# NVIDIA-NeMo/NeMo

Measured on AMD Instinct MI355X. Metric: audio-sec/s training throughput, Conformer-CTC-Large @ 1/2/4/8 MI355X, higher is better.
Workload: dtype bf16; 1 GPU; Conformer-CTC-Large bf16, batch=32x20s synthetic 16 kHz clips per GPU, 1xMI355X (BASELINE.json configs[1]); global_batch=32, parallelism=dp1

## Files before the change

nemo_amd/csrc/attention.hip:

```cpp
#include <stdlib.h>
#include "common.h"
#include "mi355x_asr.h"

typedef __attribute__((address_space(3))) void lds_void_t;
typedef const __attribute__((address_space(1))) void glb_void_t;
typedef __attribute__((ext_vector_type(4))) short s16x4;
typedef __attribute__((address_space(3))) s16x4 lds_s16x4_t;

typedef __attribute__((address_space(3))) const char lds_cchar_t;
__device__ __forceinline__ uint32_t lds_addr(const void* p) { return (uint32_t)(uintptr_t)(lds_cchar_t*)p; }

__device__ __forceinline__ void dma16(const void* src, const void* lds_base) {
  asm volatile("s_mov_b32 m0, %1\n\ts_nop 0\n\tglobal_load_lds_dwordx4 %0, off"
               :
               : "v"(src), "s"(__builtin_amdgcn_readfirstlane(lds_addr(lds_base)))
               : "memory");
}

__device__ __forceinline__ void dma4(const void* src, const void* lds_base) {
  asm volatile("s_mov_b32 m0, %1\n\ts_nop 0\n\tglobal_load_lds_dword %0, off"
               :
               : "v"(src), "s"(__builtin_amdgcn_readfirstlane(lds_addr(lds_base)))
               : "memory");
}

#define ABQ 128
#define ABK 32
#define ABAND (ABQ + ABK)
#define SG_LD 66
#define APRING 6

__device__ __forceinline__ uint32_t attn_key(const DropCfg& d, int b, int h) {
  return mix32(mix32(d.key ^ (uint32_t)(b * 0x632BE5AB)) + (uint32_t)h * 0x9E3779B9u);
}
#define ADROP_G 0x9E3779B9u
#define ADROP_KA 0x2C1B3Du
#define ADROP_KB 0x5A2D39u
__device__ __forceinline__ uint32_t adrop_rcode(uint32_t akey, uint32_t bi) { return mix32(akey + bi * 0x9E3779B9u); }
__device__ __forceinline__ uint32_t adrop_ccode(uint32_t bj) { return mix32(bj * 0x85EBCA6Bu + 0x165667B1u); }
__device__ __forceinline__ uint32_t adrop_seed(uint32_t x) { return __umul24(x, 0x846CA7u) + (x >> 13); }
__device__ __forceinline__ uint32_t adrop_y(uint32_t t) { return t ^ (t >> 15); }
__device__ __forceinline__ bool attn_keep(const DropCfg& d, uint32_t akey, int i, int j) {
  if (d.threshold == 0u) return true;
  const uint32_t seed = adrop_seed(adrop_rcode(akey, (uint32_t)i >> 2) ^ adrop_ccode((uint32_t)j >> 2));
  const uint32_t y = adrop_y(seed + (uint32_t)((i & 3) * 2 + ((j & 3) >> 1)) * ADROP_G);
  return __umul24(y, (j & 1) ? ADROP_KB : ADROP_KA) >= d.threshold;
}
__device__ __forceinline__ float attn_drop(const DropCfg& d, uint32_t akey, int i, int j) {
  return attn_keep(d, akey, i, j) ? d.scale : 0.f;
}

template <int ADK>
__device__ __forceinline__ int a_off(int r, int chunk) { return r * ADK + ((chunk ^ ((r >> 1) & 7)) << 3); }

template <int ADK>
__device__ __forceinline__ void stage_rows(const bf16_t* base, long long ld, int row0, int rmax, bf16_t* lds, int nchunks) {
  constexpr int NCH = ADK / 8;
  const int wave = threadIdx.x >> 6;
  for (int q0 = 0; q0 < nchunks; q0 += 256) {
    const int q = q0 + threadIdx.x;
    if (q0 + wave * 64 < nchunks) {
      const int r = q / NCH, ck = q % NCH;
      const int gck = ck ^ ((r >> 1) & 7);
      int gr = row0 + r;
      gr = gr < 0 ? 0 : (gr > rmax ? rmax : gr);
      const bf16_t* src = base + __mul24(gr, (int)ld) + gck * 8;
      bf16_t* dst = lds + (q0 + wave * 64) * 8;
      dma16(src, dst);
    }
  }
}
template <int ADK>
__device__ __forceinline__ void stage_v(const bf16_t* base, long long ld, int row0, int rmax, bf16_t* lds) {
  constexpr int NCH = ADK / 8;
  const int wave = threadIdx.x >> 6;
#pragma unroll
  for (int q0 = 0; q0 < 32 * NCH; q0 += 256) {
    const int q = q0 + threadIdx.x;
    const int k = q / NCH, cp = q % NCH;
    const int c = cp ^ ((k & 3) << 1);
    int gr = row0 + k;
    gr = gr > rmax ? rmax : gr;
    const bf16_t* src = base + __mul24(gr, (int)ld) + c * 8;
    bf16_t* dst = lds + (q0 + wave * 64) * 8;
    dma16(src, dst);
  }
}
template <int ADK>
__device__ __forceinline__ bf16x8 vt_frag(const bf16_t* vt, int dv0, int s, int lane) {
  const int t = lane & 15, g4 = (lane >> 4) & 1, lh = lane >> 5;
  const int col = dv0 + g4 * 16 + (t & 3) * 4;
  union { bf16x8 v; s16x4 h[2]; } u;
#pragma unroll
  for (int r = 0; r < 2; ++r) {
    const int krow = 16 * s + 8 * r + 4 * lh + (t >> 2);
    const int off = krow * ADK + (((col >> 3) ^ ((krow & 3) << 1)) << 3) + (col & 7);
    u.h[r] = __builtin_amdgcn_ds_read_tr16_b64_v4i16((lds_s16x4_t*)(vt + off));
  }
  return u.v;
}

__device__ __forceinline__ bf16x8 pack8(const float* v) {
  union { bf16x8 v; uint32_t w[4]; } u;
#pragma unroll
  for (int j = 0; j < 4; ++j) u.w[j] = pack_bf2(v[2 * j], v[2 * j + 1]);
  return u.v;
}

template <int NKK>
__device__ __forceinline__ void load_q(const bf16_t* qrow, const float* bias, bf16x8 (&out)[NKK], bool valid, int lh) {
#pragma unroll
  for (int kk = 0; kk < NKK; ++kk) {
    float v[8];
    const int k0 = kk * 16 + lh * 8;
    if (valid) {
      const u32x4 t = *reinterpret_cast<const u32x4*>(qrow + k0);
#pragma unroll
      for (int j = 0; j < 4; ++j) { v[2 * j] = __uint_as_float(t[j] << 16); v[2 * j + 1] = __uint_as_float(t[j] & 0xffff0000u); }
#pragma unroll
      for (int j = 0; j < 8; ++j) v[j] += bias[k0 + j];
    } else {
#pragma unroll
      for (int j = 0; j < 8; ++j) v[j] = 0.f;
    }
    out[kk] = pack8(v);
  }
}

template <int ADK>
__global__ __launch_bounds__(256, ADK == 64 ? 2 : 1) void relpos_flash_fwd_kernel(const bf16_t* __restrict__ qkv, long long ldq,
                                                                  const bf16_t* __restrict__ pos, long long ldp,
                                                                  const float* __restrict__ bias_u, const float* __restrict__ bias_v,
                                                                  const long long* __restrict__ len, bf16_t* __restrict__ ctx,
                                                                  bf16_t* __restrict__ ctx_lo, long long ldo,
                                                                  float* __restrict__ lse, int B, int H, int T,
                                                                  int Tp, float scale, DropCfg drop,
                                                                  const long long* __restrict__ cu) {
  drop_resolve(drop);
  constexpr int NKK = ADK / 16, NDT = ADK / 32, NCH = ADK / 8;
  __shared__ __attribute__((aligned(16))) bf16_t s_k2[2][ABK * ADK];
  __shared__ __attribute__((aligned(16))) bf16_t s_v2[2][ABK * ADK];
  __shared__ __attribute__((aligned(16))) bf16_t s_p[APRING * 32 * ADK];
  __shared__ __attribute__((aligned(16))) float s_g[4][32 * SG_LD];

  const int b = blockIdx.z, h = blockIdx.y;
  const int i0_blk = blockIdx.x * ABQ;
  const int lane = threadIdx.x & 63, wave = __builtin_amdgcn_readfirstlane(threadIdx.x >> 6);
  const int q = lane & 31, lh = lane >> 5;
  const int i = i0_blk + wave * 32 + q;
  const int L = (int)min((long long)T, len[b]);
  const bool qvalid = i < L;
  const int P = 2 * T - 1;
  const long long row0 = cu ? cu[b] : (long long)b * T;
  const int Tr = cu ? L : T;
  const int Trc = Tr > 0 ? Tr - 1 : 0;

  if (cu && i0_blk >= L) {
    if (lse && lh == 0 && i < T) lse[((long long)b * H + h) * T + i] = 0.f;
    return;
  }
  const bf16_t* qbase = qkv + row0 * ldq + h * ADK;
  const bf16_t* kbase = qbase + (ldq / 3);
  const bf16_t* vbase = qbase + 2 * (ldq / 3);
  const bf16_t* pbase = pos + h * ADK;

  bf16x8 qu[NKK], qv[NKK];
  load_q<NKK>(qbase + (long long)(i < Tr ? i : Trc) * ldq, bias_u + h * ADK, qu, i < Tr, lh);
  load_q<NKK>(qbase + (long long)(i < Tr ? i : Trc) * ldq, bias_v + h * ADK, qv, i < Tr, lh);

  f32x16 o[NDT];
#pragma unroll
  for (int t = 0; t < NDT; ++t)
#pragma unroll
    for (int r = 0; r < 16; ++r) o[t][r] = 0.f;
  float m_run = -INFINITY, l_run = 0.f;
  float* sg = s_g[wave];
  const uint32_t akey = attn_key(drop, b, h);
  const uint32_t arow = adrop_rcode(akey, (uint32_t)i >> 2), erow = (uint32_t)(i & 3) * (2u * ADROP_G);
  const float c2 = scale * 1.4426950408889634f, tau = 8.f / c2;

  const int nkt = (L + ABK - 1) / ABK;
  const int c0 = T - 1 - (i0_blk + ABQ - 1);
  if (nkt > 0) {
    stage_rows<ADK>(kbase, ldq, 0, Trc, s_k2[0], ABK * NCH);
    stage_v<ADK>(vbase, ldq, 0, Trc, s_v2[0]);
    stage_rows<ADK>(pbase, ldp, c0, P - 1, s_p, ABAND * NCH);
  }
  for (int kt = 0; kt < nkt; ++kt) {
    const int j0 = kt * ABK;
    asm volatile("s_waitcnt vmcnt(0)" ::: "memory");
    __syncthreads();
    if (kt + 1 < nkt) {
      stage_rows<ADK>(kbase, ldq, j0 + ABK, Trc, s_k2[(kt + 1) & 1], ABK * NCH);
      stage_v<ADK>(vbase, ldq, j0 + ABK, Trc, s_v2[(kt + 1) & 1]);
      stage_rows<ADK>(pbase, ldp, c0 + 32 * (kt + 5), P - 1, s_p + ((kt + 5) % APRING) * (32 * ADK), 32 * NCH);
    }
    const bf16_t* s_k = s_k2[kt & 1];
    const bf16_t* s_v = s_v2[kt & 1];
    const int slot0 = (kt + 3 - wave) % APRING, slot1 = (kt + 4 - wave) % APRING;

    f32x16 acc_s, acc_g[2];
#pragma unroll
    for (int r = 0; r < 16; ++r) { acc_s[r] = 0.f; acc_g[0][r] = 0.f; acc_g[1][r] = 0.f; }
#pragma unroll
    for (int kk = 0; kk < NKK; ++kk) {
      const bf16x8 kf = *reinterpret_cast<const bf16x8*>(s_k + a_off<ADK>(q, kk * 2 + lh));
      acc_s = __builtin_amdgcn_mfma_f32_32x32x16_bf16(kf, qu[kk], acc_s, 0, 0, 0);
#pragma unroll
      for (int gt = 0; gt < 2; ++gt) {
        const bf16x8 pf = *reinterpret_cast<const bf16x8*>(s_p + a_off<ADK>((gt ? slot1 : slot0) * 32 + q, kk * 2 + lh));
        acc_g[gt] = __builtin_amdgcn_mfma_f32_32x32x16_bf16(pf, qv[kk], acc_g[gt], 0, 0, 0);
      }
    }
#pragma unroll
    for (int gt = 0; gt < 2; ++gt)
#pragma unroll
      for (int r = 0; r < 16; ++r) sg[q * SG_LD + 32 * gt + (r & 3) + 8 * (r >> 2) + 4 * lh] = acc_g[gt][r];
    asm volatile("s_waitcnt lgkmcnt(0)" ::: "memory");
    float s[16];
    float mx = -INFINITY;
    if (j0 + ABK <= L) {
#pragma unroll
      for (int r = 0; r < 16; ++r) {
        const int rho = (r & 3) + 8 * (r >> 2) + 4 * lh;
        s[r] = acc_s[r] + sg[q * SG_LD + rho + 31 - q];
        mx = fmaxf(mx, s[r]);
      }
    } else {
#pragma unroll
      for (int r = 0; r < 16; ++r) {
        const int rho = (r & 3) + 8 * (r >> 2) + 4 * lh;
        const float bd = sg[q * SG_LD + rho + 31 - q];
        const bool ok = qvalid && (j0 + rho) < L;
        s[r] = ok ? acc_s[r] + bd : -INFINITY;
        mx = fmaxf(mx, s[r]);
      }
    }
    asm volatile("s_waitcnt lgkmcnt(0)" ::: "memory");
    mx = fmaxf(mx, __shfl_xor(mx, 32, 64));
    if (__builtin_amdgcn_ballot_w64(mx > m_run + tau) != 0ull) {
      const float m_new = fmaxf(m_run, mx);
      const float alpha = (m_new == -INFINITY) ? 1.f : __builtin_amdgcn_exp2f((m_run - m_new) * c2);
      l_run *= alpha;
#pragma unroll
      for (int r = 0; r < 16; ++r) {
#pragma unroll
        for (int t = 0; t < NDT; ++t) o[t][r] *= alpha;
      }
      m_run = m_new;
    }
    const float mc = (m_run == -INFINITY) ? 0.f : m_run * c2;
    float rs = 0.f;
#pragma unroll
    for (int r = 0; r < 16; ++r) { s[r] = __builtin_amdgcn_exp2f(fmaf(s[r], c2, -mc)); rs += s[r]; }
    rs += __shfl_xor(rs, 32, 64);
    l_run += rs;
    if (drop.threshold != 0u) {
      const uint32_t bj0 = (uint32_t)(j0 >> 2);
#pragma unroll
      for (int g = 0; g < 4; ++g) {
        const uint32_t cc0 = adrop_ccode(bj0 + 2 * g), cc1 = adrop_ccode(bj0 + 2 * g + 1);
        const uint32_t seed = adrop_seed(arow ^ (lh ? cc1 : cc0)) + erow;
#pragma unroll
        for (int cp = 0; cp < 2; ++cp) {
          const uint32_t y = adrop_y(seed + cp * ADROP_G);
          s[4 * g + 2 * cp] = __umul24(y, ADROP_KA) >= drop.threshold ? s[4 * g + 2 * cp] : 0.f;
          s[4 * g + 2 * cp + 1] = __umul24(y, ADROP_KB) >= drop.threshold ? s[4 * g + 2 * cp + 1] : 0.f;
        }
      }
    }
#pragma unroll
    for (int st = 0; st < 2; ++st) {
      const bf16x8 pb = pack8(&s[8 * st]);
#pragma unroll
      for (int dvt = 0; dvt < NDT; ++dvt) {
        const bf16x8 vf = vt_frag<ADK>(s_v, dvt * 32, st, lane);
        o[dvt] = __builtin_amdgcn_mfma_f32_32x32x16_bf16(vf, pb, o[dvt], 0, 0, 0);
      }
    }
  }

  const float inv = (qvalid && l_run > 0.f) ? (drop.threshold != 0u ? drop.scale : 1.f) / l_run : 0.f;
  __syncthreads();
  if (lse && lh == 0 && i < T) lse[((long long)b * H + h) * T + i] = qvalid ? m_run * scale + __logf(l_run) : 0.f;
#pragma unroll
  for (int half = 0; half < NDT / 2; ++half) {
#pragma unroll
  for (int dvt = 0; dvt < 2; ++dvt)
#pragma unroll
    for (int r = 0; r < 16; ++r) sg[q * SG_LD + dvt * 32 + (r & 3) + 8 * (r >> 2) + 4 * lh] = o[2 * half + dvt][r] * inv;
  asm volatile("s_waitcnt lgkmcnt(0)" ::: "memory");
#pragma unroll
  for (int it = 0; it < 4; ++it) {
    const int row = it * 8 + (lane >> 3), c8 = (lane & 7) * 8, co = half * 64 + c8;
    const int ii = i0_blk + wave * 32 + row;
    if (ii < Tr) {
      float v[8];
#pragma unroll
      for (int j = 0; j < 8; ++j) v[j] = sg[row * SG_LD + c8 + j];
      u32x4 t = {pack_bf2(v[0], v[1]), pack_bf2(v[2], v[3]), pack_bf2(v[4], v[5]), pack_bf2(v[6], v[7])};
      *reinterpret_cast<u32x4*>(ctx + (row0 + ii) * ldo + h * ADK + co) = t;
      if (ctx_lo) {
        float lo[8];
#pragma unroll
        for (int j = 0; j < 4; ++j) {
          lo[2 * j] = v[2 * j] - __uint_as_float(t[j] << 16);
          lo[2 * j + 1] = v[2 * j + 1] - __uint_as_float(t[j] & 0xffff0000u);
        }
        u32x4 tl = {pack_bf2(lo[0], lo[1]), pack_bf2(lo[2], lo[3]), pack_bf2(lo[4], lo[5]), pack_bf2(lo[6], lo[7])};
        *reinterpret_cast<u32x4*>(ctx_lo + (row0 + ii) * ldo + h * ADK + co) = tl;
      }
    }
  }
  asm volatile("s_waitcnt lgkmcnt(0)" ::: "memory");
  }
}

template <bool QB, int ADK>
__global__ __launch_bounds__(256) void attn_delta_kernel(const bf16_t* __restrict__ dO, const bf16_t* __restrict__ O,
                                                         const bf16_t* __restrict__ O_lo, float* __restrict__ delta,
                                                         const bf16_t* __restrict__ qkv, long long ldq,
                                                         const float* __restrict__ bias_u, const float* __restrict__ bias_v,
                                                         bf16_t* __restrict__ qu, bf16_t* __restrict__ qv, int B,
                                                         int H, int T, int d, const long long* __restrict__ len,
                                                         const long long* __restrict__ cu) {
  const int lane = threadIdx.x & 63;
  const long long prow = blockIdx.x * 4LL + (threadIdx.x >> 6);
  if (prow >= (long long)B * T) return;
  const int b = (int)(prow / T), i = (int)(prow - (long long)b * T);
  const bool rvalid = !cu || i < (int)min((long long)T, len[b]);
  const long long row = cu ? cu[b] + (rvalid ? i : 0) : prow;
  for (int c0 = 0; c0 < d; c0 += 512) {
    const int c = c0 + lane * 8;
    float acc = 0.f;
    if (QB && c < d && rvalid) {
      float q8[8], u8[8], v8[8], o1[8], o2[8];
      VecIO<bf16_t>::load(qkv + row * ldq + c, q8);
      VecIO<float>::load(bias_u + c, u8); VecIO<float>::load(bias_u + c + 4, &u8[4]);
      VecIO<float>::load(bias_v + c, v8); VecIO<float>::load(bias_v + c + 4, &v8[4]);
#pragma unroll
      for (int j = 0; j < 8; ++j) { o1[j] = q8[j] + u8[j]; o2[j] = q8[j] + v8[j]; }
      VecIO<bf16_t>::store(qu + row * d + c, o1);
      VecIO<bf16_t>::store(qv + row * d + c, o2);
    }
    if (c < d && rvalid) {
      const u32x4 a = *reinterpret_cast<const u32x4*>(dO + row * d + c);
      const u32x4 o = *reinterpret_cast<const u32x4*>(O + row * d + c);
#pragma unroll
      for (int j = 0; j < 4; ++j) {
        acc += __uint_as_float(a[j] << 16) * __uint_as_float(o[j] << 16);
        acc += __uint_as_float(a[j] & 0xffff0000u) * __uint_as_float(o[j] & 0xffff0000u);
      }
      if (O_lo) {
        const u32x4 l = *reinterpret_cast<const u32x4*>(O_lo + row * d + c);
        float acl = 0.f;
#pragma unroll
        for (int j = 0; j < 4; ++j) {
          acl += __uint_as_float(a[j] << 16) * __uint_as_float(l[j] << 16);
          acl += __uint_as_float(a[j] & 0xffff0000u) * __uint_as_float(l[j] & 0xffff0000u);
        }
        acc += acl;
      }
    }
    acc += __shfl_xor(acc, 1, 64); acc += __shfl_xor(acc, 2, 64); acc += __shfl_xor(acc, 4, 64);
    if (ADK == 128) acc += __shfl_xor(acc, 8, 64);
    const int h = c / ADK;
    if ((lane & (ADK / 8 - 1)) == 0 && c < d) delta[((long long)b * H + h) * T + i] = acc;
  }
}

template <int ADK>
__device__ __forceinline__ bf16x8 tr_frag(const bf16_t* img, int ra, int rb, int col0, int lane) {
  const int t = lane & 15, g4 = (lane >> 4) & 1;
  const int col = col0 + g4 * 16 + (t & 3) * 4;
  union { bf16x8 v; s16x4 h[2]; } u;
  const int r0 = ra + (t >> 2), r1 = rb + (t >> 2);
  u.h[0] = __builtin_amdgcn_ds_read_tr16_b64_v4i16((lds_s16x4_t*)(img + r0 * ADK + ((((col >> 3) ^ ((r0 >> 1) & 7))) << 3) + (col & 7)));
  u.h[1] = __builtin_amdgcn_ds_read_tr16_b64_v4i16((lds_s16x4_t*)(img + r1 * ADK + ((((col >> 3) ^ ((r1 >> 1) & 7))) << 3) + (col & 7)));
  return u.v;
}
template <int NKK>
__device__ __forceinline__ void load_rows(const bf16_t* rowp, bf16x8 (&out)[NKK], bool valid, int lh) {
#pragma unroll
  for (int kk = 0; kk < NKK; ++kk) {
    union { bf16x8 v; u32x4 w; } u;
    u.w = (u32x4){0u, 0u, 0u, 0u};
    if (valid) u.w = *reinterpret_cast<const u32x4*>(rowp + kk * 16 + lh * 8);
    out[kk] = u.v;
  }
}

template <int ADK>
__global__ __launch_bounds__(256, ADK == 64 ? 2 : 1) void relpos_flash_bwd_dq_kernel(
    const bf16_t* __restrict__ qu_g, const bf16_t* __restrict__ qv_g, const bf16_t* __restrict__ qkv, long long ldq,
    const bf16_t* __restrict__ pos, long long ldp, const long long* __restrict__ len, const bf16_t* __restrict__ dO,
    const float* __restrict__ lse, const float* __restrict__ delta, bf16_t* __restrict__ dqu_out,
    bf16_t* __restrict__ dqv_out, bf16_t* __restrict__ ds_out, bf16_t* __restrict__ dq_out, long long ld_dq,
    float* __restrict__ cs_partial, int B, int H, int T, int d, float scale, DropCfg drop,
    const long long* __restrict__ cu) {
  drop_resolve(drop);
  constexpr int NKK = ADK / 16, NDT = ADK / 32, NCH = ADK / 8;
  __shared__ __attribute__((aligned(16))) bf16_t s_k2[2][ABK * ADK];
  __shared__ __attribute__((aligned(16))) bf16_t s_v[ABK * ADK];
  __shared__ __attribute__((aligned(16))) bf16_t s_p[APRING * 32 * ADK];
  __shared__ __attribute__((aligned(16))) float s_g[4][32 * SG_LD];
  __shared__ __attribute__((aligned(16))) bf16_t s_carry[4][32 * 32];

  const int b = blockIdx.z, h = blockIdx.y;
  const int i0_blk = blockIdx.x * ABQ;
  const int lane = threadIdx.x & 63, wave = __builtin_amdgcn_readfirstlane(threadIdx.x >> 6);
  const int q = lane & 31, lh = lane >> 5;
  const int i = i0_blk + wave * 32 + q;
  const int L = (int)min((long long)T, len[b]);
  const bool qvalid = i < L;
  const int P = 2 * T - 1;
  const long long row0 = cu ? cu[b] : (long long)b * T;
  const int Tr = cu ? L : T;
  const int Trc = Tr > 0 ? Tr - 1 : 0;
  if (cu && i0_blk >= L) {
    if (dq_out && cs_partial && threadIdx.x < 2 * ADK) {
      const int uv = threadIdx.x / ADK, c = threadIdx.x % ADK;
      cs_partial[((long long)b * gridDim.x + blockIdx.x) * (2 * d) + uv * d + h * ADK + c] = 0.f;
    }
    return;
  }
  const long long rowi = row0 + (i < Tr ? i : Trc);

  const bf16_t* kbase = qkv + row0 * ldq + h * ADK + (ldq / 3);
  const bf16_t* vbase = kbase + (ldq / 3);
  const bf16_t* pbase = pos + h * ADK;

  bf16x8 qu[NKK], qv[NKK], dof[NKK];
  load_rows<NKK>(qu_g + rowi * d + h * ADK, qu, i < Tr, lh);
  load_rows<NKK>(qv_g + rowi * d + h * ADK, qv, i < Tr, lh);
  load_rows<NKK>(dO + rowi * d + h * ADK, dof, i < Tr, lh);
  float lse_i = qvalid ? lse[((long long)b * H + h) * T + i] : 1e30f;
  float dlt_i = qvalid ? delta[((long long)b * H + h) * T + i] : 0.f;
#pragma unroll
  for (int kk = 0; kk < NKK; ++kk) { asm volatile("" : "+v"(qu[kk])); asm volatile("" : "+v"(qv[kk])); asm volatile("" : "+v"(dof[kk])); }
  asm volatile("" : "+v"(lse_i), "+v"(dlt_i));

  f32x16 dqu[NDT], dqv[NDT];
#pragma unroll
  for (int t = 0; t < NDT; ++t)
#pragma unroll
    for (int r = 0; r < 16; ++r) { dqu[t][r] = 0.f; dqv[t][r] = 0.f; }
  float* sg = s_g[wave];
  const uint32_t akey = attn_key(drop, b, h);
  const uint32_t arow = adrop_rcode(akey, (uint32_t)i >> 2), erow = (uint32_t)(i & 3) * (2u * ADROP_G);
  const float c2 = scale * 1.4426950408889634f, lse2 = lse_i * 1.4426950408889634f;
  const float ks = drop.threshold != 0u ? drop.scale * scale : scale, dls = dlt_i * scale;

  const int nkt = (L + ABK - 1) / ABK;
  const int nT = (T + 31) / 32, itile = blockIdx.x * 4 + wave;
  const bool xw = ds_out != nullptr && itile < nT;
  bf16_t* xbase = ds_out + ((((long long)h * B + b) * nT + itile) * (nT + 1)) * 1024;
  u32x4* carry = reinterpret_cast<u32x4*>(s_carry[wave]);
  if (xw) { carry[lane] = (u32x4){0u, 0u, 0u, 0u}; carry[64 + lane] = (u32x4){0u, 0u, 0u, 0u}; }
  const int c0 = T - 1 - (i0_blk + ABQ - 1);
  if (nkt > 0) {
    stage_rows<ADK>(kbase, ldq, 0, Trc, s_k2[0], ABK * NCH);
    stage_rows<ADK>(vbase, ldq, 0, Trc, s_v, ABK * NCH);
    stage_rows<ADK>(pbase, ldp, c0, P - 1, s_p, ABAND * NCH);
  }
  for (int kt = 0; kt < nkt; ++kt) {
    const int j0 = kt * ABK;
    asm volatile("s_waitcnt vmcnt(0)" ::: "memory");
    __syncthreads();
    if (kt + 1 < nkt) {
      stage_rows<ADK>(kbase, ldq, j0 + ABK, Trc, s_k2[(kt + 1) & 1], ABK * NCH);
      stage_rows<ADK>(pbase, ldp, c0 + 32 * (kt + 5), P - 1, s_p + ((kt + 5) % APRING) * (32 * ADK), 32 * NCH);
    }
    const bf16_t* s_k = s_k2[kt & 1];
    const int slot0 = (kt + 3 - wave) % APRING, slot1 = (kt + 4 - wave) % APRING;

    f32x16 acc_s, acc_g[2], acc_dp;
#pragma unroll
    for (int r = 0; r < 16; ++r) { acc_s[r] = 0.f; acc_g[0][r] = 0.f; acc_g[1][r] = 0.f; acc_dp[r] = 0.f; }
#pragma unroll
    for (int kk = 0; kk < NKK; ++kk) {
      const bf16x8 kf = *reinterpret_cast<const bf16x8*>(s_k + a_off<ADK>(q, kk * 2 + lh));
      acc_s = __builtin_amdgcn_mfma_f32_32x32x16_bf16(kf, qu[kk], acc_s, 0, 0, 0);
      const bf16x8 vf = *reinterpret_cast<const bf16x8*>(s_v + a_off<ADK>(q, kk * 2 + lh));
      acc_dp = __builtin_amdgcn_mfma_f32_32x32x16_bf16(vf, dof[kk], acc_dp, 0, 0, 0);
#pragma unroll
      for (int gt = 0; gt < 2; ++gt) {
        const bf16x8 pf = *reinterpret_cast<const bf16x8*>(s_p + a_off<ADK>((gt ? slot1 : slot0) * 32 + q, kk * 2 + lh));
        acc_g[gt] = __builtin_amdgcn_mfma_f32_32x32x16_bf16(pf, qv[kk], acc_g[gt], 0, 0, 0);
      }
    }
    if (kt + 1 < nkt) {
      __syncthreads();
      stage_rows<ADK>(vbase, ldq, j0 + ABK, Trc, s_v, ABK * NCH);
    }
#pragma unroll
    for (int gt = 0; gt < 2; ++gt)
#pragma unroll
      for (int r = 0; r < 16; ++r) sg[q * SG_LD + 32 * gt + (r & 3) + 8 * (r >> 2) + 4 * lh] = acc_g[gt][r];
    asm volatile("s_waitcnt lgkmcnt(0)" ::: "memory");
    float ds[16];
    if (j0 + ABK <= L) {
#pragma unroll
      for (int r = 0; r < 16; ++r) {
        const int rho = (r & 3) + 8 * (r >> 2) + 4 * lh;
        ds[r] = __builtin_amdgcn_exp2f(fmaf(acc_s[r] + sg[q * SG_LD + rho + 31 - q], c2, -lse2));
      }
    } else {
#pragma unroll
      for (int r = 0; r < 16; ++r) {
        const int rho = (r & 3) + 8 * (r >> 2) + 4 * lh;
        const float bd = sg[q * SG_LD + rho + 31 - q];
        ds[r] = (j0 + rho) < L ? __builtin_amdgcn_exp2f(fmaf(acc_s[r] + bd, c2, -lse2)) : 0.f;
      }
    }
    asm volatile("s_waitcnt lgkmcnt(0)" ::: "memory");
    if (drop.threshold != 0u) {
      const uint32_t bj0 = (uint32_t)(j0 >> 2);
#pragma unroll
      for (int g = 0; g < 4; ++g) {
        const uint32_t cc0 = adrop_ccode(bj0 + 2 * g), cc1 = adrop_ccode(bj0 + 2 * g + 1);
        const uint32_t seed = adrop_seed(arow ^ (lh ? cc1 : cc0)) + erow;
#pragma unroll
        for (int cp = 0; cp < 2; ++cp) {
          const uint32_t y = adrop_y(seed + cp * ADROP_G);
          const int r0 = 4 * g + 2 * cp;
          const float x0 = __umul24(y, ADROP_KA) >= drop.threshold ? acc_dp[r0] : 0.f;
          const float x1 = __umul24(y, ADROP_KB) >= drop.threshold ? acc_dp[r0 + 1] : 0.f;
          ds[r0] *= fmaf(x0, ks, -dls);
          ds[r0 + 1] *= fmaf(x1, ks, -dls);
        }
      }
    } else {
#pragma unroll
      for (int r = 0; r < 16; ++r) ds[r] *= fmaf(acc_dp[r], ks, -dls);
    }
#pragma unroll
    for (int st = 0; st < 2; ++st) {
      const bf16x8 db = pack8(&ds[8 * st]);
#pragma unroll
      for (int dkt = 0; dkt < NDT; ++dkt) {
        const bf16x8 kt_f = tr_frag<ADK>(s_k, 16 * st + 4 * lh, 16 * st + 8 + 4 * lh, dkt * 32, lane);
        dqu[dkt] = __builtin_amdgcn_mfma_f32_32x32x16_bf16(kt_f, db, dqu[dkt], 0, 0, 0);
      }
    }
    {
      const float2 z = make_float2(0.f, 0.f);
#pragma unroll
      for (int w2 = 0; w2 < 16; ++w2) *reinterpret_cast<float2*>(sg + q * SG_LD + 32 * lh + 2 * w2) = z;
    }
    asm volatile("s_waitcnt lgkmcnt(0)" ::: "memory");
#pragma unroll
    for (int r = 0; r < 16; ++r) sg[q * SG_LD + (r & 3) + 8 * (r >> 2) + 4 * lh + 31 - q] = ds[r];
    asm volatile("s_waitcnt lgkmcnt(0)" ::: "memory");
#pragma unroll
    for (int s4 = 0; s4 < 4; ++s4) {
      float gv[8];
#pragma unroll
      for (int e = 0; e < 8; ++e) gv[e] = sg[q * SG_LD + 16 * s4 + 8 * lh + e];
      const bf16x8 gb = pack8(gv);
#pragma unroll
      for (int dkt = 0; dkt < NDT; ++dkt) {
        const int ra = (s4 < 2 ? slot0 : slot1) * 32 + 16 * (s4 & 1) + 8 * lh;
        const bf16x8 pt_f = tr_frag<ADK>(s_p, ra, ra + 4, dkt * 32, lane);
        dqv[dkt] = __builtin_amdgcn_mfma_f32_32x32x16_bf16(pt_f, gb, dqv[dkt], 0, 0, 0);
      }
    }
    asm volatile("s_waitcnt lgkmcnt(0)" ::: "memory");
    if (xw) {
#pragma unroll
      for (int it2 = 0; it2 < 2; ++it2) {
        const int row = it2 * 16 + (lane >> 2), c8 = (lane & 3) * 8;
        float lo[8], hi[8];
#pragma unroll
        for (int e = 0; e < 8; ++e) { lo[e] = sg[row * SG_LD + c8 + e]; hi[e] = sg[row * SG_LD + 32 + c8 + e]; }
        const u32x4 cw = carry[it2 * 64 + lane];
        u32x4 t = {pack_bf2(lo[0], lo[1]) | cw.x, pack_bf2(lo[2], lo[3]) | cw.y, pack_bf2(lo[4], lo[5]) | cw.z,
                   pack_bf2(lo[6], lo[7]) | cw.w};
        *reinterpret_cast<u32x4*>(xbase + (long long)kt * 1024 + it2 * 512 + lane * 8) = t;
        carry[it2 * 64 + lane] = (u32x4){pack_bf2(hi[0], hi[1]), pack_bf2(hi[2], hi[3]), pack_bf2(hi[4], hi[5]), pack_bf2(hi[6], hi[7])};
      }
      asm volatile("s_waitcnt lgkmcnt(0)" ::: "memory");
    }
  }
  if (xw) {
#pragma unroll
    for (int it2 = 0; it2 < 2; ++it2)
      *reinterpret_cast<u32x4*>(xbase + (long long)nkt * 1024 + it2 * 512 + lane * 8) = carry[it2 * 64 + lane];
  }

  __syncthreads();
  constexpr int NH = NDT / 2;
  float keep[NH][4][8], cs[2][NH][8];
#pragma unroll
  for (int hf = 0; hf < NH; ++hf)
#pragma unroll
    for (int j = 0; j < 8; ++j) { cs[0][hf][j] = 0.f; cs[1][hf][j] = 0.f; }
#pragma unroll
  for (int pass = 0; pass < 2; ++pass) {
    bf16_t* outp = pass == 0 ? dqu_out : dqv_out;
#pragma unroll
    for (int hf = 0; hf < NH; ++hf) {
#pragma unroll
    for (int dkt = 0; dkt < 2; ++dkt)
#pragma unroll
      for (int r = 0; r < 16; ++r)
        sg[q * SG_LD + dkt * 32 + (r & 3) + 8 * (r >> 2) + 4 * lh] = qvalid ? (pass == 0 ? dqu[2 * hf + dkt][r] : dqv[2 * hf + dkt][r]) : 0.f;
    asm volatile("s_waitcnt lgkmcnt(0)" ::: "memory");
#pragma unroll
    for (int it = 0; it < 4; ++it) {
      const int row = it * 8 + (lane >> 3), c8 = (lane & 7) * 8, co = hf * 64 + c8;
      const int ii = i0_blk + wave * 32 + row;
      if (ii < Tr) {
        float v[8];
#pragma unroll
        for (int j = 0; j < 8; ++j) v[j] = sg[row * SG_LD + c8 + j];
        if (outp) {
          u32x4 t = {pack_bf2(v[0], v[1]), pack_bf2(v[2], v[3]), pack_bf2(v[4], v[5]), pack_bf2(v[6], v[7])};
          *reinterpret_cast<u32x4*>(outp + (row0 + ii) * d + h * ADK + co) = t;
        }
        if (dq_out) {
#pragma unroll
          for (int j = 0; j < 8; ++j) cs[pass][hf][j] += v[j];
          if (pass == 0) {
#pragma unroll
            for (int j = 0; j < 8; ++j) keep[hf][it][j] = v[j];
          } else {
#pragma unroll
            for (int j = 0; j < 8; ++j) v[j] += keep[hf][it][j];
            u32x4 t = {pack_bf2(v[0], v[1]), pack_bf2(v[2], v[3]), pack_bf2(v[4], v[5]), pack_bf2(v[6], v[7])};
            *reinterpret_cast<u32x4*>(dq_out + (row0 + ii) * ld_dq + h * ADK + co) = t;
          }
        }
      }
    }
    asm volatile("s_waitcnt lgkmcnt(0)" ::: "memory");
    }
  }
  if (dq_out && cs_partial) {
#pragma unroll
    for (int pass = 0; pass < 2; ++pass)
#pragma unroll
      for (int hf = 0; hf < NH; ++hf)
#pragma unroll
      for (int j = 0; j < 8; ++j) {
        float v = cs[pass][hf][j];
        v += __shfl_xor(v, 8, 64); v += __shfl_xor(v, 16, 64); v += __shfl_xor(v, 32, 64);
        cs[pass][hf][j] = v;
      }
    if (lane < 8) {
#pragma unroll
      for (int pass = 0; pass < 2; ++pass)
#pragma unroll
        for (int hf = 0; hf < NH; ++hf)
#pragma unroll
        for (int j = 0; j < 8; ++j) sg[pass * ADK + hf * 64 + lane * 8 + j] = cs[pass][hf][j];
    }
    __syncthreads();
    if (threadIdx.x < 2 * ADK) {
      const int uv = threadIdx.x / ADK, c = threadIdx.x % ADK;
      const float t = (s_g[0][threadIdx.x] + s_g[1][threadIdx.x]) + (s_g[2][threadIdx.x] + s_g[3][threadIdx.x]);
      cs_partial[((long long)b * gridDim.x + blockIdx.x) * (2 * d) + uv * d + h * ADK + c] = t;
    }
  }
}

template <int ADK>
__global__ __launch_bounds__(256, ADK == 64 ? 2 : 1) void relpos_flash_bwd_dkv_kernel(
    const bf16_t* __restrict__ qu_g, const bf16_t* __restrict__ qv_g, const bf16_t* __restrict__ qkv, long long ldq,
    const bf16_t* __restrict__ pos, long long ldp, const long long* __restrict__ len, const bf16_t* __restrict__ dO,
    const float* __restrict__ lse, const float* __restrict__ delta, bf16_t* __restrict__ dqkv, long long ldd, int B, int H,
    int T, int Tp, int d, float scale, DropCfg drop, const long long* __restrict__ cu) {
  drop_resolve(drop);
  constexpr int NKK = ADK / 16, NDT = ADK / 32, NCH = ADK / 8;
  constexpr int STAGE_BYTES = 2 * 3 * 32 * ADK * 2 + APRING * 32 * ADK * 2 + 2 * 2 * 32 * 4;
  constexpr int OUT_BYTES = 4 * 32 * SG_LD * 4;
  __shared__ __attribute__((aligned(16))) char s_raw[STAGE_BYTES > OUT_BYTES ? STAGE_BYTES : OUT_BYTES];
  bf16_t* const s_q3 = reinterpret_cast<bf16_t*>(s_raw);
  bf16_t* const s_p = reinterpret_cast<bf16_t*>(s_raw + 2 * 3 * 32 * ADK * 2);
  float* const s_ld = reinterpret_cast<float*>(s_raw + 2 * 3 * 32 * ADK * 2 + APRING * 32 * ADK * 2);

  const int b = blockIdx.z, h = blockIdx.y;
  const int j0_blk = blockIdx.x * ABQ;
  const int lane = threadIdx.x & 63, wave = __builtin_amdgcn_readfirstlane(threadIdx.x >> 6);
  const int q = lane & 31, lh = lane >> 5;
  const int j = j0_blk + wave * 32 + q;
  const int L = (int)min((long long)T, len[b]);
  const bool kvalid = j < L;
  const int P = 2 * T - 1;
  const long long row0 = cu ? cu[b] : (long long)b * T;
  const int Tr = cu ? L : T;
  const int Trc = Tr > 0 ? Tr - 1 : 0;
  if (cu && j0_blk >= L) return;
  const long long rowj = row0 + (j < Tr ? j : Trc);
  const bf16_t* kbase = qkv + (ldq / 3) + h * ADK;
  const bf16_t* pbase = pos + h * ADK;
  const uint32_t akey = attn_key(drop, b, h);
  const uint32_t acol = adrop_ccode((uint32_t)j >> 2), ecol = (uint32_t)((j & 3) >> 1) * ADROP_G;
  const uint32_t klane = (j & 1) ? ADROP_KB : ADROP_KA;
  const float dscale = drop.threshold != 0u ? drop.scale : 1.f;

  bf16x8 kf[NKK], vf[NKK];
  load_rows<NKK>(kbase + rowj * ldq, kf, j < Tr, lh);
  load_rows<NKK>(kbase + (ldq / 3) + rowj * ldq, vf, j < Tr, lh);

#pragma unroll
  for (int kk = 0; kk < NKK; ++kk) { asm volatile("" : "+v"(kf[kk])); asm volatile("" : "+v"(vf[kk])); }
  f32x16 dk_acc[NDT], dv_acc[NDT];
#pragma unroll
  for (int t = 0; t < NDT; ++t)
#pragma unroll
    for (int r = 0; r < 16; ++r) { dk_acc[t][r] = 0.f; dv_acc[t][r] = 0.f; }

  const int nqt = (L + 31) / 32;
  const bf16_t* qub = qu_g + row0 * d + h * ADK;
  const bf16_t* qvb = qv_g + row0 * d + h * ADK;
  const bf16_t* dob = dO + row0 * d + h * ADK;
  const int cb0 = T - 1 + j0_blk - 31;
  auto stage_q = [&](int i0, int buf) {
    bf16_t* dst = s_q3 + buf * (3 * 32 * ADK);
    stage_rows<ADK>(qub, d, i0, Trc, dst, 32 * NCH);
    stage_rows<ADK>(qvb, d, i0, Trc, dst + 32 * ADK, 32 * NCH);
    stage_rows<ADK>(dob, d, i0, Trc, dst + 2 * 32 * ADK, 32 * NCH);
    if (wave == 0) {
      int ii = i0 + (lane & 31);
      ii = ii < T ? ii : T - 1;
      dma4((lane < 32 ? lse : delta) + ((long long)b * H + h) * T + ii, s_ld + buf * 64);
    }
  };
  if (nqt > 0) {
    stage_q(0, 0);
    stage_rows<ADK>(pbase, ldp, cb0, P - 1, s_p, ABAND * NCH);
  }
  for (int qt = 0; qt < nqt; ++qt) {
    const int i0 = qt * 32;
    asm volatile("s_waitcnt vmcnt(0)" ::: "memory");
    __syncthreads();
    if (qt + 1 < nqt) {
      stage_q(i0 + 32, (qt + 1) & 1);
      stage_rows<ADK>(pbase, ldp, cb0 - 32 * (qt + 1), P - 1, s_p + ((6 * 1024 - (qt + 1)) % APRING) * (32 * ADK), 32 * NCH);
    }
    const bf16_t* s_qu = s_q3 + (qt & 1) * (3 * 32 * ADK);
    const bf16_t* s_qv = s_qu + 32 * ADK;
    const bf16_t* s_do = s_qu + 2 * 32 * ADK;
    const float* s_lse = s_ld + (qt & 1) * 64;
    const float* s_dlt = s_lse + 32;
    const int slot0 = (6 * 1024 - qt + wave) % APRING, slot1 = (6 * 1024 - qt + wave + 1) % APRING;

    f32x16 acc_s, acc_g[2], acc_dp;
#pragma unroll
    for (int r = 0; r < 16; ++r) { acc_s[r] = 0.f; acc_g[0][r] = 0.f; acc_g[1][r] = 0.f; acc_dp[r] = 0.f; }
#pragma unroll
    for (int kk = 0; kk < NKK; ++kk) {
      const bf16x8 quf = *reinterpret_cast<const bf16x8*>(s_qu + a_off<ADK>(q, kk * 2 + lh));
      acc_s = __builtin_amdgcn_mfma_f32_32x32x16_bf16(quf, kf[kk], acc_s, 0, 0, 0);
      const bf16x8 dof = *reinterpret_cast<const bf16x8*>(s_do + a_off<ADK>(q, kk * 2 + lh));
      acc_dp = __builtin_amdgcn_mfma_f32_32x32x16_bf16(dof, vf[kk], acc_dp, 0, 0, 0);
      const bf16x8 qvf = *reinterpret_cast<const bf16x8*>(s_qv + a_off<ADK>(q, kk * 2 + lh));
#pragma unroll
      for (int ct = 0; ct < 2; ++ct) {
        const bf16x8 pf = *reinterpret_cast<const bf16x8*>(s_p + a_off<ADK>((ct ? slot1 : slot0) * 32 + q, kk * 2 + lh));
        acc_g[ct] = __builtin_amdgcn_mfma_f32_32x32x16_bf16(qvf, pf, acc_g[ct], 0, 0, 0);
      }
    }
    float pd[16], ds[16];
    uint32_t w4[4] = {0xffffffffu, 0xffffffffu, 0xffffffffu, 0xffffffffu};
#pragma unroll
    for (int r = 0; r < 16; ++r) {
      if ((r & 3) == 0 && drop.threshold != 0u) {
        const uint32_t rr0 = adrop_rcode(akey, (uint32_t)(i0 >> 2) + 2 * (r >> 2));
        const uint32_t rr1 = adrop_rcode(akey, (uint32_t)(i0 >> 2) + 2 * (r >> 2) + 1);
        const uint32_t seed = adrop_seed((lh ? rr1 : rr0) ^ acol) + ecol;
#pragma unroll
        for (int c = 0; c < 4; ++c) w4[c] = __umul24(adrop_y(seed + c * (2u * ADROP_G)), klane);
      }
      const int rho = (r & 3) + 8 * (r >> 2) + 4 * lh;
      const int sl = 31 + q - rho;
      const float g0 = __shfl(acc_g[0][r], lh * 32 + (sl & 31), 64);
      const float g1 = __shfl(acc_g[1][r], lh * 32 + (sl & 31), 64);
      const float bd = sl < 32 ? g0 : g1;
      const int ii = i0 + rho;
      const bool ok = kvalid && ii < L;
      const float p = ok ? __expf((acc_s[r] + bd) * scale - s_lse[rho]) : 0.f;
      const bool keep = w4[r & 3] >= drop.threshold;
      pd[r] = keep ? p : 0.f;
      ds[r] = p * fmaf(keep ? acc_dp[r] : 0.f, dscale, -s_dlt[rho]);
    }
#pragma unroll
    for (int st = 0; st < 2; ++st) {
      const bf16x8 pb = pack8(&pd[8 * st]);
      const bf16x8 db = pack8(&ds[8 * st]);
      const int ra = 16 * st + 4 * lh, rb = 16 * st + 8 + 4 * lh;
#pragma unroll
      for (int t2 = 0; t2 < NDT; ++t2) {
        const bf16x8 dot_f = tr_frag<ADK>(s_do, ra, rb, t2 * 32, lane);
        dv_acc[t2] = __builtin_amdgcn_mfma_f32_32x32x16_bf16(dot_f, pb, dv_acc[t2], 0, 0, 0);
        const bf16x8 qut_f = tr_frag<ADK>(s_qu, ra, rb, t2 * 32, lane);
        dk_acc[t2] = __builtin_amdgcn_mfma_f32_32x32x16_bf16(qut_f, db, dk_acc[t2], 0, 0, 0);
      }
    }
  }
  __syncthreads();

  float* st_ = reinterpret_cast<float*>(s_raw) + wave * (32 * SG_LD);
#pragma unroll
  for (int pass = 0; pass < 2 * (NDT / 2); ++pass) {
    const int kind = pass / (NDT / 2), hf = pass % (NDT / 2);
#pragma unroll
    for (int t2 = 0; t2 < 2; ++t2)
#pragma unroll
      for (int r = 0; r < 16; ++r)
        st_[q * SG_LD + t2 * 32 + (r & 3) + 8 * (r >> 2) + 4 * lh] =
            kind == 0 ? dk_acc[2 * hf + t2][r] * scale : dv_acc[2 * hf + t2][r] * dscale;
    asm volatile("s_waitcnt lgkmcnt(0)" ::: "memory");
#pragma unroll
    for (int it = 0; it < 4; ++it) {
      const int row = it * 8 + (lane >> 3), c8 = (lane & 7) * 8;
      const int jj = j0_blk + wave * 32 + row;
      if (jj < Tr) {
        float v[8];
#pragma unroll
        for (int e = 0; e < 8; ++e) v[e] = st_[row * SG_LD + c8 + e];
        u32x4 t = {pack_bf2(v[0], v[1]), pack_bf2(v[2], v[3]), pack_bf2(v[4], v[5]), pack_bf2(v[6], v[7])};
        *reinterpret_cast<u32x4*>(dqkv + (row0 + jj) * ldd + (kind + 1) * (ldd / 3) + h * ADK + hf * 64 + c8) = t;
      }
    }
    asm volatile("s_waitcnt lgkmcnt(0)" ::: "memory");
  }
}

__device__ __forceinline__ bf16x8 tr_frag32(const bf16_t* img, int ra, int rb, int lane) {
  const int t = lane & 15, g4 = (lane >> 4) & 1;
  const int col = g4 * 16 + (t & 3) * 4;
  union { bf16x8 v; s16x4 h[2]; } u;
  u.h[0] = __builtin_amdgcn_ds_read_tr16_b64_v4i16((lds_s16x4_t*)(img + (ra + (t >> 2)) * 32 + col));
  u.h[1] = __builtin_amdgcn_ds_read_tr16_b64_v4i16((lds_s16x4_t*)(img + (rb + (t >> 2)) * 32 + col));
  return u.v;
}

template <int ADK>
__global__ __launch_bounds__(256, ADK == 64 ? 2 : 1) void relpos_flash_bwd_dpos_kernel(
    const bf16_t* __restrict__ qv_g, const bf16_t* __restrict__ x_g, const long long* __restrict__ len,
    float* __restrict__ dpos, long long ldd, float* __restrict__ partial, int B, int H, int T, int d, int bchunk,
    const long long* __restrict__ cu) {
  constexpr int NDT = ADK / 32, NCH = ADK / 8;
  __shared__ __attribute__((aligned(16))) bf16_t s_x[4][2][2 * 1024];
  __shared__ __attribute__((aligned(16))) bf16_t s_qv[4][2][32 * ADK];

  const int nT = (T + 31) / 32;
  const int dg = 2 * (int)blockIdx.x - (nT - 1);
  const int h = blockIdx.y;
  const int b_begin = blockIdx.z * bchunk, b_end = min(B, b_begin + bchunk);
  const int lane = threadIdx.x & 63, wave = __builtin_amdgcn_readfirstlane(threadIdx.x >> 6);
  const int q = lane & 31, lh = lane >> 5;
  const int P = 2 * T - 1;
  const int cmin = T - 32 + 32 * dg;
  const int it_lo = max(0, -dg - 1), it_hi = min(nT, nT - dg + 1);

  f32x16 dp_acc[2][NDT];
#pragma unroll
  for (int t = 0; t < NDT; ++t)
#pragma unroll
    for (int r = 0; r < 16; ++r) { dp_acc[0][t][r] = 0.f; dp_acc[1][t][r] = 0.f; }

  const int npairs = it_hi - it_lo;
  const int nitems = (b_end - b_begin) * npairs;
  auto issue = [&](int b, int it, int buf) {
    const int s0 = it + dg;
    const int sl0 = min(max(s0, 0), nT), sl1 = min(max(s0 + 1, 0), nT);
    const bf16_t* base = x_g + ((((long long)h * B + b) * nT + it) * (nT + 1)) * 1024;
    bf16_t* sx = s_x[wave][buf];
    bf16_t* sqv = s_qv[wave][buf];
#pragma unroll
    for (int k2 = 0; k2 < 2; ++k2) {
      dma16((base + sl0 * 1024 + k2 * 512 + lane * 8), (sx + k2 * 512));
      dma16((base + sl1 * 1024 + k2 * 512 + lane * 8), (sx + 1024 + k2 * 512));
    }
    const int Lb = cu ? (int)min((long long)T, len[b]) : T;
    const bf16_t* qb = qv_g + (cu ? (Lb > 0 ? cu[b] : 0LL) : (long long)b * T) * d + h * ADK;
    const int grmax = Lb > 0 ? Lb - 1 : 0;
#pragma unroll
    for (int k4 = 0; k4 < 32 * NCH / 64; ++k4) {
      const int cq = k4 * 64 + lane;
      const int r = cq / NCH, ck = cq % NCH;
      int gr = 32 * it + r;
      gr = gr > grmax ? grmax : gr;
      dma16((qb + __mul24(gr, d) + ((ck ^ ((r >> 1) & 7)) << 3)), (sqv + k4 * 512));
    }
  };
  auto advance = [&](int& b, int& it, int steps) {
    it += steps;
    while (it >= it_hi) { it -= npairs; ++b; }
  };
  uint32_t xaddr, qaddr[2][NDT][2];
  {
    const int t = lane & 15, g4 = (lane >> 4) & 1;
    xaddr = lds_addr(&s_x[wave][0][0]) + (uint32_t)(((8 * lh + (t >> 2)) * 32 + g4 * 16 + (t & 3) * 4) * 2);
#pragma unroll
    for (int st = 0; st < 2; ++st)
#pragma unroll
      for (int dkt = 0; dkt < NDT; ++dkt)
#pragma unroll
        for (int hf = 0; hf < 2; ++hf) {
          const int r = 16 * st + 8 * lh + 4 * hf + (t >> 2), col = dkt * 32 + g4 * 16 + (t & 3) * 4;
          qaddr[st][dkt][hf] = lds_addr(&s_qv[wave][0][0]) + (uint32_t)((r * ADK + (((col >> 3) ^ ((r >> 1) & 7)) << 3) + (col & 7)) * 2);
        }
  }
  int cb = b_begin, cit = it_lo;
  advance(cb, cit, wave);
  int nb = cb, nit = cit;
  if (wave < nitems) issue(cb, cit, 0);
  int buf = 0;
  for (int item = wave; item < nitems; item += 4, buf ^= 1, advance(cb, cit, 4)) {
    if (item + 4 < nitems) {
      nb = cb; nit = cit; advance(nb, nit, 4);
      issue(nb, nit, buf ^ 1);
      if constexpr (ADK == 64) asm volatile("s_waitcnt vmcnt(8)" ::: "memory");
      else asm volatile("s_waitcnt vmcnt(12)" ::: "memory");
    } else asm volatile("s_waitcnt vmcnt(0)" ::: "memory");
    const int b = cb;
    const int it = cit, s0 = it + dg;
    const int L = (int)min((long long)T, len[b]);
    const int nkt = (L + 31) / 32;
    const bool v0 = s0 >= 0 && s0 <= nkt, v1 = s0 + 1 >= 0 && s0 + 1 <= nkt;
    if (32 * it >= L || !(v0 || v1)) continue;
    const uint32_t m0 = v0 ? 0xffffffffu : 0u, m1 = v1 ? 0xffffffffu : 0u;
    const uint32_t xa = xaddr + buf * 4096u, qoff = buf * (uint32_t)(32 * ADK * 2);
#pragma unroll
    for (int st = 0; st < 2; ++st) {
      union { bf16x8 v; s16x4 h[2]; u32x4 w; } af[2], bq[NDT];
      asm volatile(
          "ds_read_b64_tr_b16 %0, %8\n\t"
          "ds_read_b64_tr_b16 %1, %8 offset:256\n\t"
// ... 233 lines not shown
```

Measured before the change: 18390 audio-sec/s.

## Reuse relpos band block across key tiles and write ds directly from registers

```diff
diff --git a/nemo_amd/csrc/attention.hip b/nemo_amd/csrc/attention.hip
--- a/nemo_amd/csrc/attention.hip
+++ b/nemo_amd/csrc/attention.hip
@@ -56,7 +56,7 @@
 template <int ADK>
 __device__ __forceinline__ void stage_rows(const bf16_t* base, long long ld, int row0, int rmax, bf16_t* lds, int nchunks) {
   constexpr int NCH = ADK / 8;
-  const int wave = threadIdx.x >> 6;
+  const int wave = __builtin_amdgcn_readfirstlane(threadIdx.x >> 6);
   for (int q0 = 0; q0 < nchunks; q0 += 256) {
     const int q = q0 + threadIdx.x;
     if (q0 + wave * 64 < nchunks) {
@@ -64,7 +64,7 @@
       const int gck = ck ^ ((r >> 1) & 7);
       int gr = row0 + r;
       gr = gr < 0 ? 0 : (gr > rmax ? rmax : gr);
-      const bf16_t* src = base + __mul24(gr, (int)ld) + gck * 8;
+      const bf16_t* src = base + (__mul24(gr, (int)ld) + gck * 8);
       bf16_t* dst = lds + (q0 + wave * 64) * 8;
       dma16(src, dst);
     }
@@ -73,7 +73,7 @@
 template <int ADK>
 __device__ __forceinline__ void stage_v(const bf16_t* base, long long ld, int row0, int rmax, bf16_t* lds) {
   constexpr int NCH = ADK / 8;
-  const int wave = threadIdx.x >> 6;
+  const int wave = __builtin_amdgcn_readfirstlane(threadIdx.x >> 6);
 #pragma unroll
   for (int q0 = 0; q0 < 32 * NCH; q0 += 256) {
     const int q = q0 + threadIdx.x;
@@ -81,7 +81,7 @@
     const int c = cp ^ ((k & 3) << 1);
     int gr = row0 + k;
     gr = gr > rmax ? rmax : gr;
-    const bf16_t* src = base + __mul24(gr, (int)ld) + c * 8;
+    const bf16_t* src = base + (__mul24(gr, (int)ld) + c * 8);
     bf16_t* dst = lds + (q0 + wave * 64) * 8;
     dma16(src, dst);
   }
@@ -124,6 +124,17 @@
       for (int j = 0; j < 8; ++j) v[j] = 0.f;
     }
     out[kk] = pack8(v);
+  }
+}
+
+template <int ADK>
+__device__ __forceinline__ void band_block(const bf16_t* s_p, int slot, const bf16x8 (&qv)[ADK / 16], int q, int lh, f32x16& acc) {
+#pragma unroll
+  for (int r = 0; r < 16; ++r) acc[r] = 0.f;
+#pragma unroll
+  for (int kk = 0; kk < ADK / 16; ++kk) {
+    const bf16x8 pf = *reinterpret_cast<const bf16x8*>(s_p + a_off<ADK>(slot * 32 + q, kk * 2 + lh));
+    acc = __builtin_amdgcn_mfma_f32_32x32x16_bf16(pf, qv[kk], acc, 0, 0, 0);
   }
 }
 
@@ -181,6 +192,7 @@
 
   const int nkt = (L + ABK - 1) / ABK;
   const int c0 = T - 1 - (i0_blk + ABQ - 1);
+  f32x16 g_carry;
   if (nkt > 0) {
     stage_rows<ADK>(kbase, ldq, 0, Trc, s_k2[0], ABK * NCH);
     stage_v<ADK>(vbase, ldq, 0, Trc, s_v2[0]);
@@ -200,18 +212,21 @@
     const int slot0 = (kt + 3 - wave) % APRING, slot1 = (kt + 4 - wave) % APRING;
 
     f32x16 acc_s, acc_g[2];
-#pragma unroll
-    for (int r = 0; r < 16; ++r) { acc_s[r] = 0.f; acc_g[0][r] = 0.f; acc_g[1][r] = 0.f; }
+    if (kt == 0) {
+      band_block<ADK>(s_p, slot0, qv, q, lh, acc_g[0]);
+    } else {
+      acc_g[0] = g_carry;
+    }
+#pragma unroll
+    for (int r = 0; r < 16; ++r) { acc_s[r] = 0.f; acc_g[1][r] = 0.f; }
 #pragma unroll
     for (int kk = 0; kk < NKK; ++kk) {
       const bf16x8 kf = *reinterpret_cast<const bf16x8*>(s_k + a_off<ADK>(q, kk * 2 + lh));
       acc_s = __builtin_amdgcn_mfma_f32_32x32x16_bf16(kf, qu[kk], acc_s, 0, 0, 0);
-#pragma unroll
-      for (int gt = 0; gt < 2; ++gt) {
-        const bf16x8 pf = *reinterpret_cast<const bf16x8*>(s_p + a_off<ADK>((gt ? slot1 : slot0) * 32 + q, kk * 2 + lh));
-        acc_g[gt] = __builtin_amdgcn_mfma_f32_32x32x16_bf16(pf, qv[kk], acc_g[gt], 0, 0, 0);
-      }
-    }
+      const bf16x8 pf = *reinterpret_cast<const bf16x8*>(s_p + a_off<ADK>(slot1 * 32 + q, kk * 2 + lh));
+      acc_g[1] = __builtin_amdgcn_mfma_f32_32x32x16_bf16(pf, qv[kk], acc_g[1], 0, 0, 0);
+    }
+    g_carry = acc_g[1];
 #pragma unroll
     for (int gt = 0; gt < 2; ++gt)
 #pragma unroll
@@ -404,7 +419,6 @@
   __shared__ __attribute__((aligned(16))) bf16_t s_v[ABK * ADK];
   __shared__ __attribute__((aligned(16))) bf16_t s_p[APRING * 32 * ADK];
   __shared__ __attribute__((aligned(16))) float s_g[4][32 * SG_LD];
-  __shared__ __attribute__((aligned(16))) bf16_t s_carry[4][32 * 32];
 
   const int b = blockIdx.z, h = blockIdx.y;
   const int i0_blk = blockIdx.x * ABQ;
@@ -455,8 +469,8 @@
   const int nT = (T + 31) / 32, itile = blockIdx.x * 4 + wave;
   const bool xw = ds_out != nullptr && itile < nT;
   bf16_t* xbase = ds_out + ((((long long)h * B + b) * nT + itile) * (nT + 1)) * 1024;
-  u32x4* carry = reinterpret_cast<u32x4*>(s_carry[wave]);
-  if (xw) { carry[lane] = (u32x4){0u, 0u, 0u, 0u}; carry[64 + lane] = (u32x4){0u, 0u, 0u, 0u}; }
+  u32x4 carry[2] = {(u32x4){0u, 0u, 0u, 0u}, (u32x4){0u, 0u, 0u, 0u}};
+  f32x16 g_carry;
   const int c0 = T - 1 - (i0_blk + ABQ - 1);
   if (nkt > 0) {
     stage_rows<ADK>(kbase, ldq, 0, Trc, s_k2[0], ABK * NCH);
@@ -475,20 +489,23 @@
     const int slot0 = (kt + 3 - wave) % APRING, slot1 = (kt + 4 - wave) % APRING;
 
     f32x16 acc_s, acc_g[2], acc_dp;
-#pragma unroll
-    for (int r = 0; r < 16; ++r) { acc_s[r] = 0.f; acc_g[0][r] = 0.f; acc_g[1][r] = 0.f; acc_dp[r] = 0.f; }
+    if (kt == 0) {
+      band_block<ADK>(s_p, slot0, qv, q, lh, acc_g[0]);
+    } else {
+      acc_g[0] = g_carry;
+    }
+#pragma unroll
+    for (int r = 0; r < 16; ++r) { acc_s[r] = 0.f; acc_g[1][r] = 0.f; acc_dp[r] = 0.f; }
 #pragma unroll
     for (int kk = 0; kk < NKK; ++kk) {
       const bf16x8 kf = *reinterpret_cast<const bf16x8*>(s_k + a_off<ADK>(q, kk * 2 + lh));
       acc_s = __builtin_amdgcn_mfma_f32_32x32x16_bf16(kf, qu[kk], acc_s, 0, 0, 0);
       const bf16x8 vf = *reinterpret_cast<const bf16x8*>(s_v + a_off<ADK>(q, kk * 2 + lh));
       acc_dp = __builtin_amdgcn_mfma_f32_32x32x16_bf16(vf, dof[kk], acc_dp, 0, 0, 0);
-#pragma unroll
-      for (int gt = 0; gt < 2; ++gt) {
-        const bf16x8 pf = *reinterpret_cast<const bf16x8*>(s_p + a_off<ADK>((gt ? slot1 : slot0) * 32 + q, kk * 2 + lh));
-        acc_g[gt] = __builtin_amdgcn_mfma_f32_32x32x16_bf16(pf, qv[kk], acc_g[gt], 0, 0, 0);
-      }
-    }
+      const bf16x8 pf = *reinterpret_cast<const bf16x8*>(s_p + a_off<ADK>(slot1 * 32 + q, kk * 2 + lh));
+      acc_g[1] = __builtin_amdgcn_mfma_f32_32x32x16_bf16(pf, qv[kk], acc_g[1], 0, 0, 0);
+    }
+    g_carry = acc_g[1];
     if (kt + 1 < nkt) {
       __syncthreads();
       stage_rows<ADK>(vbase, ldq, j0 + ABK, Trc, s_v, ABK * NCH);
@@ -557,35 +574,26 @@
       float gv[8];
 #pragma unroll
       for (int e = 0; e < 8; ++e) gv[e] = sg[q * SG_LD + 16 * s4 + 8 * lh + e];
-      const bf16x8 gb = pack8(gv);
+      union { bf16x8 v; u32x4 w; } gb;
+      gb.v = pack8(gv);
 #pragma unroll
       for (int dkt = 0; dkt < NDT; ++dkt) {
         const int ra = (s4 < 2 ? slot0 : slot1) * 32 + 16 * (s4 & 1) + 8 * lh;
         const bf16x8 pt_f = tr_frag<ADK>(s_p, ra, ra + 4, dkt * 32, lane);
-        dqv[dkt] = __builtin_amdgcn_mfma_f32_32x32x16_bf16(pt_f, gb, dqv[dkt], 0, 0, 0);
+        dqv[dkt] = __builtin_amdgcn_mfma_f32_32x32x16_bf16(pt_f, gb.v, dqv[dkt], 0, 0, 0);
+      }
+      if (s4 < 2) {
+        if (xw) *reinterpret_cast<u32x4*>(xbase + (long long)kt * 1024 + q * 32 + 16 * s4 + 8 * lh) = gb.w | carry[s4];
+      } else {
+        carry[s4 - 2] = gb.w;
       }
     }
     asm volatile("s_waitcnt lgkmcnt(0)" ::: "memory");
-    if (xw) {
-#pragma unroll
-      for (int it2 = 0; it2 < 2; ++it2) {
-        const int row = it2 * 16 + (lane >> 2), c8 = (lane & 3) * 8;
-        float lo[8], hi[8];
-#pragma unroll
-        for (int e = 0; e < 8; ++e) { lo[e] = sg[row * SG_LD + c8 + e]; hi[e] = sg[row * SG_LD + 32 + c8 + e]; }
-        const u32x4 cw = carry[it2 * 64 + lane];
-        u32x4 t = {pack_bf2(lo[0], lo[1]) | cw.x, pack_bf2(lo[2], lo[3]) | cw.y, pack_bf2(lo[4], lo[5]) | cw.z,
-                   pack_bf2(lo[6], lo[7]) | cw.w};
-        *reinterpret_cast<u32x4*>(xbase + (long long)kt * 1024 + it2 * 512 + lane * 8) = t;
-        carry[it2 * 64 + lane] = (u32x4){pack_bf2(hi[0], hi[1]), pack_bf2(hi[2], hi[3]), pack_bf2(hi[4], hi[5]), pack_bf2(hi[6], hi[7])};
-      }
-      asm volatile("s_waitcnt lgkmcnt(0)" ::: "memory");
-    }
   }
   if (xw) {
 #pragma unroll
-    for (int it2 = 0; it2 < 2; ++it2)
-      *reinterpret_cast<u32x4*>(xbase + (long long)nkt * 1024 + it2 * 512 + lane * 8) = carry[it2 * 64 + lane];
+    for (int s2 = 0; s2 < 2; ++s2)
+      *reinterpret_cast<u32x4*>(xbase + (long long)nkt * 1024 + q * 32 + 16 * s2 + 8 * lh) = carry[s2];
   }
 
   __syncthreads();
@@ -775,9 +783,8 @@
       }
       const int rho = (r & 3) + 8 * (r >> 2) + 4 * lh;
       const int sl = 31 + q - rho;
-      const float g0 = __shfl(acc_g[0][r], lh * 32 + (sl & 31), 64);
-      const float g1 = __shfl(acc_g[1][r], lh * 32 + (sl & 31), 64);
-      const float bd = sl < 32 ? g0 : g1;
+      const float gsel = q >= 31 - rho ? acc_g[0][r] : acc_g[1][r];
+      const float bd = __shfl(gsel, lh * 32 + (sl & 31), 64);
       const int ii = i0 + rho;
       const bool ok = kvalid && ii < L;
       const float p = ok ? __expf((acc_s[r] + bd) * scale - s_lse[rho]) : 0.f;
```

Result: no change. 18460 audio-sec/s (median of 6 runs) (+0.4%).
